# ReactiveBayes/RxInfer.jl

Hardware: NVIDIA H100
Metric: gaussian_messages_per_sec_batched_lgssm_d4_T1000 (higher is better)
Workload: dtype f32

## Files before the change

rxinfer.jl_b200/csrc/rxg_gain.cuh:

```cuda
#pragma once
#include <cooperative_groups.h>

#include "rxg_lgssm_common.cuh"

namespace rxg {
namespace cg = cooperative_groups;

constexpr int GS_CTAS = 8;
constexpr int GS_THREADS = 128;
constexpr int GS_NT = GS_CTAS * GS_THREADS;

struct ScanWs {
    double* fel;
    double* ftot;
    double* bel;
    double* btot;
};

template <int R, int C>
__device__ __forceinline__ Mat<double, R, C> ldcg_d(const double* p) {
    Mat<double, R, C> o;
#pragma unroll
    for (int i = 0; i < R * C; ++i) o.a[i] = __ldcg(p + i);
    return o;
}
template <int R, int C>
__device__ __forceinline__ Mat<double, R, C> ld_soa_d(const double* p, size_t n, size_t i) {
    Mat<double, R, C> o;
#pragma unroll
    for (int c = 0; c < R * C; ++c) o.a[c] = __ldcg(p + (size_t)c * n + i);
    return o;
}
template <int R, int C>
__device__ __forceinline__ void st_soa_d(double* p, size_t n, size_t i, const Mat<double, R, C>& A) {
#pragma unroll
    for (int c = 0; c < R * C; ++c) p[(size_t)c * n + i] = A.a[c];
}

template <int N, int K>
__device__ __forceinline__ Mat<double, N, K> solve_general(Mat<double, N, N> Mx, Mat<double, N, K> Rh) {
#pragma unroll
    for (int c = 0; c < N; ++c) {
        int p = c;
        double best = fabs(Mx(c, c));
#pragma unroll
        for (int r = c + 1; r < N; ++r) {
            const double v = fabs(Mx(r, c));
            if (v > best) { best = v; p = r; }
        }
#pragma unroll
        for (int r = c + 1; r < N; ++r) {
            if (r == p) {
#pragma unroll
                for (int j = c; j < N; ++j) { const double t = Mx(c, j); Mx(c, j) = Mx(r, j); Mx(r, j) = t; }
#pragma unroll
                for (int j = 0; j < K; ++j) { const double t = Rh(c, j); Rh(c, j) = Rh(r, j); Rh(r, j) = t; }
            }
        }
        const double inv = 1.0 / Mx(c, c);
#pragma unroll
        for (int r = c + 1; r < N; ++r) {
            const double f = Mx(r, c) * inv;
#pragma unroll
            for (int j = c + 1; j < N; ++j) Mx(r, j) = fma(-f, Mx(c, j), Mx(r, j));
#pragma unroll
            for (int j = 0; j < K; ++j) Rh(r, j) = fma(-f, Rh(c, j), Rh(r, j));
        }
    }
    Mat<double, N, K> X;
#pragma unroll
    for (int c = N - 1; c >= 0; --c) {
        const double inv = 1.0 / Mx(c, c);
#pragma unroll
        for (int k = 0; k < K; ++k) {
            double s = Rh(c, k);
#pragma unroll
            for (int j = c + 1; j < N; ++j) s = fma(-Mx(c, j), X(j, k), s);
            X(c, k) = s * inv;
        }
    }
    return X;
}

template <int D>
struct FwdEl {
    Mat<double, D, D> A, C, J;
};
template <int D>
struct BwdEl {
    Mat<double, D, D> E, L;
};

template <int D>
__device__ __forceinline__ FwdEl<D> fwd_identity() {
    FwdEl<D> e;
    e.A = identity<double, D>();
#pragma unroll
    for (int i = 0; i < D * D; ++i) { e.C.a[i] = 0.0; e.J.a[i] = 0.0; }
    return e;
}
template <int D>
__device__ __forceinline__ void fwd_store(double* p, size_t n, size_t i, const FwdEl<D>& e) {
    st_soa_d<D, D>(p, n, i, e.A);
    st_soa_d<D, D>(p + (size_t)D * D * n, n, i, e.C);
    st_soa_d<D, D>(p + (size_t)2 * D * D * n, n, i, e.J);
}
template <int D>
__device__ __forceinline__ FwdEl<D> fwd_load(const double* p, size_t n, size_t i) {
    FwdEl<D> e;
    e.A = ld_soa_d<D, D>(p, n, i);
    e.C = ld_soa_d<D, D>(p + (size_t)D * D * n, n, i);
    e.J = ld_soa_d<D, D>(p + (size_t)2 * D * D * n, n, i);
    return e;
}
template <int D, bool C_ONLY>
__device__ __forceinline__ FwdEl<D> fwd_combine(const FwdEl<D>& ei, const FwdEl<D>& ej) {
    Mat<double, D, D> Mx = mul(ei.C, ej.J);
#pragma unroll
    for (int i = 0; i < D; ++i) Mx(i, i) += 1.0;
    Mat<double, D, 2 * D> Rh;
#pragma unroll
    for (int i = 0; i < D; ++i)
#pragma unroll
        for (int j = 0; j < D; ++j) { Rh(i, j) = ei.A(i, j); Rh(i, D + j) = ei.C(i, j); }
    Mat<double, D, 2 * D> X = solve_general<D, 2 * D>(Mx, Rh);
    Mat<double, D, D> X1, X2;
#pragma unroll
    for (int i = 0; i < D; ++i)
#pragma unroll
        for (int j = 0; j < D; ++j) { X1(i, j) = X(i, j); X2(i, j) = X(i, D + j); }
    FwdEl<D> o;
    Mat<double, D, D> T2 = mul(ej.A, X2);
    o.C = sym_mul_nt_add(T2, ej.A, ej.C);
    if (!C_ONLY) {
        o.A = mul(ej.A, X1);
        Mat<double, D, D> JX = mul(ej.J, X1);
        Mat<double, D, D> AtJX = mul_tn(ei.A, JX);
#pragma unroll
        for (int i = 0; i < D; ++i)
#pragma unroll
            for (int j = 0; j <= i; ++j) {
                const double s = 0.5 * (AtJX(i, j) + AtJX(j, i)) + ei.J(i, j);
                o.J(i, j) = s; o.J(j, i) = s;
            }
    }
    return o;
}

template <int D>
__device__ __forceinline__ void bwd_store(double* p, size_t n, size_t i, const BwdEl<D>& e) {
    st_soa_d<D, D>(p, n, i, e.E);
    st_soa_d<D, D>(p + (size_t)D * D * n, n, i, e.L);
}
template <int D>
__device__ __forceinline__ BwdEl<D> bwd_load(const double* p, size_t n, size_t i) {
    BwdEl<D> e;
    e.E = ld_soa_d<D, D>(p, n, i);
    e.L = ld_soa_d<D, D>(p + (size_t)D * D * n, n, i);
    return e;
}
template <int D, bool L_ONLY>
__device__ __forceinline__ BwdEl<D> bwd_combine(const BwdEl<D>& early, const BwdEl<D>& late) {
    BwdEl<D> o;
    Mat<double, D, D> EL = mul(early.E, late.L);
    o.L = sym_mul_nt_add(EL, early.E, early.L);
    if (!L_ONLY) o.E = mul(early.E, late.E);
    return o;
}

template <int D, int M>
__global__ void __cluster_dims__(GS_CTAS, 1, 1) __launch_bounds__(GS_THREADS, 1)
gain_scan_kernel(const __grid_constant__ ModelF<D, M> mdl, GainWs ws, ScanWs sw, int T, int transition_first,
                 float* __restrict__ cov_shared_out, int* __restrict__ bad_out, const uint8_t* __restrict__ tmask,
                 const float* __restrict__ useq) {
    using TB = Tab<D, M>;
    cg::cluster_group cluster = cg::this_cluster();
    const int g = (int)cluster.block_rank() * GS_THREADS + (int)threadIdx.x;
    const int E = (T + GS_NT - 1) / GS_NT;
    const int k0 = g * E, k1 = min(k0 + E, T);
    constexpr int FE = 3 * D * D, BE = 2 * D * D;
    bool bad = false;

    const Mat<double, D, D> A = load_const<double, D, D>(mdl.A), P = load_const<double, D, D>(mdl.P);
    const Mat<double, M, D> B = load_const<double, M, D>(mdl.B);
    const Mat<double, M, M> Q = load_const<double, M, M>(mdl.Q);

    {
        FwdEl<D> acc = fwd_identity<D>();
        if (k0 < k1) {
            FwdEl<D> gen;
            {
                Mat<double, M, D> BP = mul(B, P);
                Mat<double, M, M> Sinn = sym_mul_nt_add(BP, B, Q);
                Chol<double, M> ch = cholesky<double, M, false>(Sinn, bad);
                Mat<double, D, M> V = solve_right_Lt(transpose(BP), ch.L);
                Mat<double, D, M> K = solve_right_L(V, ch.L);
                Mat<double, D, D> IKB = identity<double, D>();
#pragma unroll
                for (int i = 0; i < D; ++i)
#pragma unroll
                    for (int j = 0; j < D; ++j)
#pragma unroll
                        for (int k = 0; k < M; ++k) IKB(i, j) -= K(i, k) * B(k, j);
                gen.A = mul(IKB, A);
                gen.C = sym_downdate(P, V);
                Mat<double, M, D> BA = mul(B, A);
                Mat<double, M, D> Wm;
#pragma unroll
                for (int c = 0; c < D; ++c) {
                    Vec<double, M> col;
#pragma unroll
                    for (int r = 0; r < M; ++r) col(r) = BA(r, c);
                    Vec<double, M> z = solve_L(ch.L, col);
#pragma unroll
                    for (int r = 0; r < M; ++r) Wm(r, c) = z(r);
                }
                Mat<double, D, D> Z;
#pragma unroll
                for (int i = 0; i < D * D; ++i) Z.a[i] = 0.0;
                gen.J = sym_mul_nt_add(transpose(Wm), transpose(Wm), Z);
            }
            for (int k = k0; k < k1; ++k) {
                if (k == 0) {
                    Mat<double, D, D> S = load_const<double, D, D>(mdl.S0);
                    if (transition_first) { Mat<double, D, D> AS = mul(A, S); S = sym_mul_nt_add(AS, A, P); }
                    FwdEl<D> first;
#pragma unroll
                    for (int i = 0; i < D * D; ++i) { first.A.a[i] = 0.0; first.J.a[i] = 0.0; }
                    if (!tmask || tmask[0] != 0) {
                        Mat<double, M, D> BS = mul(B, S);
                        Mat<double, M, M> Sinn = sym_mul_nt_add(BS, B, Q);
                        Chol<double, M> ch = cholesky<double, M, false>(Sinn, bad);
                        Mat<double, D, M> V = solve_right_Lt(transpose(BS), ch.L);
                        first.C = sym_downdate(S, V);
                    } else {
                        first.C = S;
                    }
                    acc = first;
                } else {
                    const bool obs_k = !tmask || tmask[k] != 0;
                    if (obs_k) {
                        acc = (k == k0) ? gen : fwd_combine<D, false>(acc, gen);
                    } else {
                        FwdEl<D> miss;
                        miss.A = A; miss.C = P;
#pragma unroll
                        for (int i = 0; i < D * D; ++i) miss.J.a[i] = 0.0;
                        acc = (k == k0) ? miss : fwd_combine<D, false>(acc, miss);
                    }
                }
                if (E > 1) fwd_store<D>(sw.fel, T, k, acc);
            }
        }
        fwd_store<D>(sw.ftot, GS_NT, g, acc);
    }
    cluster.sync();
    int cur = 0;
    for (int off = 1; off < GS_NT; off <<= 1) {
        const double* src = sw.ftot + (size_t)cur * GS_NT * FE;
        double* dst = sw.ftot + (size_t)(cur ^ 1) * GS_NT * FE;
        FwdEl<D> mine = fwd_load<D>(src, GS_NT, g);
        if (g >= off && (g - off) * E < T && k0 < T) {
            FwdEl<D> prev = fwd_load<D>(src, GS_NT, g - off);
            mine = fwd_combine<D, false>(prev, mine);
        }
        fwd_store<D>(dst, GS_NT, g, mine);
        cluster.sync();
        cur ^= 1;
    }
    {
        const double* tot = sw.ftot + (size_t)cur * GS_NT * FE;
        if (E == 1) {
            if (g < T) store_d(ws.Sf + (size_t)g * D * D, ld_soa_d<D, D>(tot + (size_t)D * D * GS_NT, GS_NT, g));
        } else if (k0 < k1) {
            if (g == 0) {
                for (int k = k0; k < k1; ++k)
                    store_d(ws.Sf + (size_t)k * D * D, ld_soa_d<D, D>(sw.fel + (size_t)D * D * T, T, k));
            } else {
                const FwdEl<D> excl = fwd_load<D>(tot, GS_NT, g - 1);
                for (int k = k0; k < k1; ++k) {
                    const FwdEl<D> pk = fwd_load<D>(sw.fel, T, k);
                    store_d(ws.Sf + (size_t)k * D * D, fwd_combine<D, true>(excl, pk).C);
                }
            }
        }
    }
    cluster.sync();
    for (int t = g; t < T; t += GS_NT) {
        const Mat<double, D, D> Sf = ldcg_d<D, D>(ws.Sf + (size_t)t * D * D);
        Mat<double, D, D> Sp;
        if (t > 0) {
            Mat<double, D, D> Sfm = ldcg_d<D, D>(ws.Sf + (size_t)(t - 1) * D * D);
            Mat<double, D, D> AS = mul(A, Sfm);
            Sp = sym_mul_nt_add(AS, A, P);
        } else {
            Sp = load_const<double, D, D>(mdl.S0);
            if (transition_first) { Mat<double, D, D> AS = mul(A, Sp); Sp = sym_mul_nt_add(AS, A, P); }
        }
        const bool obs_t = !tmask || tmask[t] != 0;
        {
            Mat<double, D, M> K;
            Mat<double, M, M> Li;
            double cconst = 0.0;
#pragma unroll
            for (int i = 0; i < D * M; ++i) K.a[i] = 0.0;
#pragma unroll
            for (int i = 0; i < M * M; ++i) Li.a[i] = 0.0;
            if (obs_t) {
                Mat<double, M, D> BS = mul(B, Sp);
                Mat<double, M, M> Sinn = sym_mul_nt_add(BS, B, Q);
                Chol<double, M> ch = cholesky<double, M, true>(Sinn, bad);
                Mat<double, D, M> V = solve_right_Lt(transpose(BS), ch.L);
                K = solve_right_L(V, ch.L);
#pragma unroll
                for (int j = 0; j < M; ++j) {
                    Li(j, j) = ch.L(j, j);
// ... 2 lines not shown
                        double sacc = 0.0;
#pragma unroll
                        for (int k = j; k < i; ++k) sacc -= ch.L(i, k) * Li(k, j);
                        Li(i, j) = sacc * ch.L(i, i);
                    }
                }
                cconst = M * RXG_HALF_LOG_2PI - ch.neg_half_logdet;
            }
            Mat<double, D, D> IKB = identity<double, D>();
#pragma unroll
            for (int i = 0; i < D; ++i)
#pragma unroll
                for (int j = 0; j < D; ++j)
#pragma unroll
                    for (int k = 0; k < M; ++k) IKB(i, j) -= K(i, k) * B(k, j);
            Mat<double, D, D> F = (t > 0 || transition_first) ? mul(IKB, A) : IKB;
            float* rec = ws.fwd + (size_t)t * TB::FWD_REC;
            store_f(rec + TB::F_OFF, F);
            store_f(rec + TB::K_OFF, K);
            store_f(rec + TB::LI_OFF, Li);
            rec[TB::C_OFF] = (float)cconst;
            Vec<double, D> uu, gf;
#pragma unroll
            for (int i = 0; i < D; ++i) uu(i) = (double)(useq ? useq[(size_t)t * D + i] : mdl.u[i]);
            gf = mulv(IKB, uu);
            if (!(t > 0 || transition_first)) {
#pragma unroll
                for (int i = 0; i < D; ++i) gf(i) = 0.0;
            }
            store_fv(rec + TB::GF_OFF, gf);
            store_f(ws.sf + (size_t)t * TB::SF_REC, Sf);
        }
        float* brec = ws.bwd + (size_t)t * TB::BWD_REC;
        BwdEl<D> be;
        Vec<double, D> gb;
#pragma unroll
        for (int i = 0; i < D; ++i) gb(i) = 0.0;
        if (t < T - 1) {
            Mat<double, D, D> AS = mul(A, Sf);
            Mat<double, D, D> Sp1 = sym_mul_nt_add(AS, A, P);
            Chol<double, D> ch = cholesky<double, D, false>(Sp1, bad);
            Mat<double, D, D> U = solve_right_Lt(transpose(AS), ch.L);
            be.E = solve_right_L(U, ch.L);
            be.L = sym_downdate(Sf, U);
            Mat<double, D, D> Em = identity<double, D>();
            Mat<double, D, D> GA = mul(be.E, A);
#pragma unroll
            for (int i = 0; i < D * D; ++i) Em.a[i] -= GA.a[i];
            store_f(brec + TB::E_OFF, Em);
            store_f(brec + TB::G_OFF, be.E);
            Vec<double, D> uu;
#pragma unroll
            for (int i = 0; i < D; ++i) uu(i) = -(double)(useq ? useq[(size_t)(t + 1) * D + i] : mdl.u[i]);
            gb = mulv(be.E, uu);
        } else {
#pragma unroll
            for (int i = 0; i < D * D; ++i) be.E.a[i] = 0.0;
            be.L = Sf;
            store_f(brec + TB::E_OFF, identity<double, D>());
            store_f(brec + TB::G_OFF, be.E);
        }
        store_fv(brec + TB::GB_OFF, gb);
        bwd_store<D>(sw.bel, T, t, be);
    }
    cluster.sync();
    {
        BwdEl<D> acc;
        acc.E = identity<double, D>();
#pragma unroll
        for (int i = 0; i < D * D; ++i) acc.L.a[i] = 0.0;
        for (int r = k0; r < k1; ++r) {
            const int t = T - 1 - r;
            const BwdEl<D> el = bwd_load<D>(sw.bel, T, t);
            acc = (r == k0) ? el : bwd_combine<D, false>(el, acc);
            if (E > 1) bwd_store<D>(sw.bel, T, t, acc);
        }
        bwd_store<D>(sw.btot, GS_NT, g, acc);
    }
    cluster.sync();
    cur = 0;
    for (int off = 1; off < GS_NT; off <<= 1) {
        const double* src = sw.btot + (size_t)cur * GS_NT * BE;
        double* dst = sw.btot + (size_t)(cur ^ 1) * GS_NT * BE;
        BwdEl<D> mine = bwd_load<D>(src, GS_NT, g);
        if (g >= off && k0 < T) {
            BwdEl<D> prev = bwd_load<D>(src, GS_NT, g - off);
            mine = bwd_combine<D, false>(mine, prev);
        }
        bwd_store<D>(dst, GS_NT, g, mine);
        cluster.sync();
        cur ^= 1;
    }
    {
        const double* tot = sw.btot + (size_t)cur * GS_NT * BE;
        BwdEl<D> excl;
        if (E > 1 && g > 0 && k0 < k1) excl = bwd_load<D>(tot, GS_NT, g - 1);
        for (int r = k0; r < k1; ++r) {
            const int t = T - 1 - r;
            Mat<double, D, D> Ss;
            if (E == 1) {
                Ss = ld_soa_d<D, D>(tot + (size_t)D * D * GS_NT, GS_NT, g);
            } else {
                const BwdEl<D> pr = bwd_load<D>(sw.bel, T, t);
                Ss = (g == 0) ? pr.L : bwd_combine<D, true>(pr, excl).L;
            }
            store_f(ws.bwd + (size_t)t * TB::BWD_REC + TB::SS_OFF, Ss);
            if (cov_shared_out) store_f(cov_shared_out + (size_t)t * D * D, Ss);
        }
    }
    if (bad) atomicOr(bad_out, 1);
}

}
```

rxinfer.jl_b200/csrc/rxg_lgssm.cu:

```cuda
#include <math.h>
#include <stdlib.h>

#include <utility>

#include "rxg_chain_step.cuh"
#include "rxg_gain.cuh"
#include "rxg_internal.h"
#include "rxg_linalg.cuh"
#include "rxg_lgssm_cluster.cuh"
#include "rxg_lgssm_common.cuh"
#include "rxg_lgssm_shared.cuh"
#include "rxg_lgssm_seg.cuh"
#include "rxg_sweep_select.h"

namespace rxg {

template <int D, int M, bool PER_CHAIN, bool SMOOTH, bool USEQ = false>
__global__ void __launch_bounds__(128)
lgssm_chain_kernel(const __grid_constant__ ModelF<D, M> mdl, PerChainPtrs pc,
                   const float* __restrict__ y, const uint8_t* __restrict__ mask,
                   float* __restrict__ mean, float* __restrict__ cov, float* __restrict__ nle,
                   int32_t* __restrict__ status, int T, int64_t batch, int transition_first,
                   const float* __restrict__ useq = nullptr, int64_t ustride = 0, int uchain = 0) {
    const int64_t b = (int64_t)blockIdx.x * blockDim.x + threadIdx.x;
// ... 388 lines not shown
    launched = false;
    if constexpr (D * D <= 16 && M >= D) {
        using CT = ClusterTab<D, M>;
        bool offset = false;
        for (int i = 0; i < D; ++i) offset |= (mdl.u[i] != 0.f);
        const bool aligned = (((uintptr_t)c.y | (uintptr_t)c.mean | (uintptr_t)c.cov) & 15) == 0;
        if (!c.smooth || c.nle || c.useq || offset || c.mean0_chain || c.batch % 32 != 0 || !aligned ||
            ctx->opt[RXG_OPT_SWEEP_VARIANT] != 0 || ctx->opt[RXG_OPT_FORCE_CPT] != 0)
            return RXG_OK;
        const size_t smem = CT::smem_bytes(c.T);
        int smem_max = 0;
        RXG_CUDA(ctx, cudaDeviceGetAttribute(&smem_max, cudaDevAttrMaxSharedMemoryPerBlockOptin, ctx->device));
        if (smem > (size_t)smem_max) return RXG_OK;
        const bool peer = c.po.n_mean > 0 || c.po.n_cov > 0;
        auto kern = peer ? lgssm_cluster_sweep_kernel<D, M, true> : lgssm_cluster_sweep_kernel<D, M, false>;
        RXG_CUDA(ctx, cudaFuncSetAttribute(kern, cudaFuncAttributeMaxDynamicSharedMemorySize, (int)smem));
        cudaLaunchConfig_t cfg = {};
        cudaLaunchAttribute attr[1];
        attr[0].id = cudaLaunchAttributeClusterDimension;
        attr[0].val.clusterDim.x = CL_CTAS;
        attr[0].val.clusterDim.y = 1;
        attr[0].val.clusterDim.z = 1;
        cfg.gridDim = dim3((unsigned)(c.batch / 32 * CL_CTAS));
        cfg.blockDim = dim3(32 * CL_WARPS);
        cfg.dynamicSmemBytes = smem;
        cfg.stream = ctx->stream;
        cfg.attrs = attr;
        cfg.numAttrs = 1;
        int nclusters = 0;
        RXG_CUDA(ctx, cudaOccupancyMaxActiveClusters(&nclusters, kern, &cfg));
        if (nclusters < 1) return RXG_OK;

        const int spc = CT::spc(c.T);
        cluster_tables_kernel<D, M><<<1, 256, 0, ctx->stream>>>(ws, cl_tab, c.T, spc);
        if (ctx->profile) cudaEventRecord(ctx->ev[1], ctx->stream);
        RXG_CUDA(ctx, cudaLaunchKernelEx(&cfg, kern, (const float*)ws.fwd, (const float*)ws.bwd, (const float*)cl_tab, c.y,
                                         c.mean, c.cov, c.T, c.batch, write_cov, mdl, c.po));
        if (ctx->profile) cudaEventRecord(ctx->ev[2], ctx->stream);
        ctx->launches += 2;
        c.fused_peer_stores = peer;
        launched = true;
        return check_cuda(ctx, cudaGetLastError(), "lgssm_cluster_sweep_kernel launch");
    }
    return RXG_OK;
}

template <int D, int M>
static int run_shared_family(rxg_ctx* ctx, LgssmCall& c) {
    using TB = Tab<D, M>;
    ModelF<D, M> mdl = {};
    fill_model<D, M>(mdl, c);
    const size_t T = (size_t)c.T;
    size_t off = 0;
    auto carve = [&](size_t bytes) { size_t o = off; off += (bytes + 255) / 256 * 256; return o; };
    const size_t o_fwd = carve(T * TB::FWD_REC * sizeof(float));
    const size_t o_bwd = carve(T * TB::BWD_REC * sizeof(float));
    const size_t o_sf = carve(T * TB::SF_REC * sizeof(float));
    const size_t o_Sp = carve(T * D * D * sizeof(double));
    const size_t o_Sf = carve(T * D * D * sizeof(double));
    const size_t o_Cc = carve(T * D * D * sizeof(double));
    const size_t o_Gd = carve(T * D * D * sizeof(double));
    const size_t o_fel = carve(T * 3 * D * D * sizeof(double));
    const size_t o_ftot = carve((size_t)2 * GS_NT * 3 * D * D * sizeof(double));
    const size_t o_bel = carve(T * 2 * D * D * sizeof(double));
    const size_t o_btot = carve((size_t)2 * GS_NT * 2 * D * D * sizeof(double));
    using ST = SegTab<D, M>;
    const size_t nseg = (T + ST::L - 1) / ST::L;
    const size_t o_srec_t = carve(T * ST::REC * sizeof(float)), o_snrec = carve(T * ST::NREC * sizeof(float));
    const size_t o_ssrec = carve(nseg * ST::SREC * sizeof(float));
    const size_t o_ctab = carve(c.want_cov_table ? T * D * D * sizeof(float) : 0);
    const size_t o_cl = carve(ClusterTab<D, M>::table_floats(c.T) * sizeof(float));
    char* base = (char*)workspace(ctx, off);
    if (!base) return RXG_ERR_CUDA;
    GainWs ws;
    ws.fwd = (float*)(base + o_fwd); ws.bwd = (float*)(base + o_bwd); ws.sf = (float*)(base + o_sf);
    ws.Sp = (double*)(base + o_Sp); ws.Sf = (double*)(base + o_Sf);
    ws.Cc = (double*)(base + o_Cc); ws.Gd = (double*)(base + o_Gd);
    ScanWs sw;
    sw.fel = (double*)(base + o_fel); sw.ftot = (double*)(base + o_ftot);
    sw.bel = (double*)(base + o_bel); sw.btot = (double*)(base + o_btot);

    const int tf = (c.flags & RXG_TRANSITION_FIRST) ? 1 : 0;
    const bool cov_shared = (c.flags & RXG_COV_SHARED_OUT) != 0;
    c.cov_table = (c.want_cov_table && c.smooth) ? (float*)(base + o_ctab) : nullptr;
    if (ctx->profile) cudaEventRecord(ctx->ev[0], ctx->stream);
    float* cov_once = (cov_shared && c.cov && c.smooth) ? c.cov : (c.smooth ? c.cov_table : nullptr);
    const float* useq_tab = c.useq_chain ? nullptr : c.useq;
    if (ctx->opt[RXG_OPT_GAIN_SEQ] != 0) {
        gain_riccati_seq<D, M><<<1, 32, 0, ctx->stream>>>(mdl, ws, c.T, tf, bad_flag(ctx), c.tmask);
        gain_tables<D, M><<<(c.T + 63) / 64, 64, 0, ctx->stream>>>(mdl, ws, c.T, tf, bad_flag(ctx), c.tmask, useq_tab);
        ctx->launches += 2;
        if (c.smooth) {
            gain_smooth_seq<D, M><<<1, 32, 0, ctx->stream>>>(ws, c.T, cov_once);
            ctx->launches += 1;
        }
    } else {
        gain_scan_kernel<D, M><<<GS_CTAS, GS_THREADS, 0, ctx->stream>>>(mdl, ws, sw, c.T, tf, cov_once, bad_flag(ctx), c.tmask,
                                                                          useq_tab);
        ctx->launches += 1;
    }
    if (!c.smooth && cov_shared && c.cov) {
        const int n = c.T * D * D;
        copy_table_kernel<<<(n + 255) / 256, 256, 0, ctx->stream>>>(ws.sf, TB::SF_REC, D * D, c.T, c.cov);
        ctx->launches += 1;
    }
    int rc = check_cuda(ctx, cudaGetLastError(), "gain table kernels launch");
    if (rc != RXG_OK) return rc;
    if (c.ev_tables) RXG_CUDA(ctx, cudaEventRecord(c.ev_tables, ctx->stream));
    if (c.tables_only) return RXG_OK;
    const int write_cov = (c.cov != nullptr && !cov_shared) ? 1 : 0;
    bool launched = false;
    rc = launch_cluster_if_eligible<D, M>(ctx, c, mdl, ws, (float*)(base + o_cl), write_cov, launched);
    if (rc != RXG_OK || launched) return rc;
    const long long variant = ctx->opt[RXG_OPT_SWEEP_VARIANT];
    if (variant == 3 && !c.useq && seg_sweep_eligible<D, M>(c)) {
        SegWs sgw;
        sgw.rec = (float*)(base + o_srec_t); sgw.nrec = (float*)(base + o_snrec); sgw.srec = (float*)(base + o_ssrec);
        return launch_seg<D, M>(ctx, c, mdl, ws, sgw, write_cov, variant == 3);
    }
    SweepQuery q = {};
    q.d = D;
    q.m = M;
    q.batch = c.batch;
    q.sm_count = ctx->sm_count;
    q.force_cpt = ctx->opt[RXG_OPT_FORCE_CPT];
    q.aligned16 = (((uintptr_t)c.y | (uintptr_t)c.mean | (uintptr_t)c.cov | (uintptr_t)c.nle | (uintptr_t)c.mean0_chain |
                    (uintptr_t)(c.useq_chain ? c.useq : nullptr)) & 15) == 0;
    q.smooth = c.smooth;
    q.evid = c.nle != nullptr;
    for (int i = 0; i < D; ++i) q.offset |= (mdl.u[i] != 0.f);
    q.input = !c.useq ? InputSeq::none : (c.useq_chain ? InputSeq::per_chain : InputSeq::shared);
// ... 56 lines not shown
```

rxinfer.jl_b200/csrc/rxg_lgssm_cluster.cuh:

```cuda
#pragma once
#include <cooperative_groups.h>

#include "rxg_lgssm_common.cuh"
#include "rxg_lgssm_shared.cuh"

namespace rxg {

constexpr int CL_CTAS = 8;
constexpr int CL_WARPS = 8;
constexpr int CL_L = 16;

template <int D, int M>
struct ClusterTab {
    static constexpr int FK = pad4(D * D) + pad4(D * M);
    static constexpr int EG = 2 * pad4(D * D);
    static constexpr int REC = 2 * pad4(D * D);
    static constexpr int PSI_OFF = pad4(D * D);
    static_assert(Tab<D, M>::F_OFF == 0 && Tab<D, M>::K_OFF == pad4(D * D) && Tab<D, M>::E_OFF == 0 &&
                      Tab<D, M>::G_OFF == pad4(D * D),
                  "the staged prefixes are the first FK / EG floats of the gain records");

    static __host__ __device__ int spc(int T) { return ((T + CL_L - 1) / CL_L + CL_CTAS - 1) / CL_CTAS; }
    static size_t table_floats(int T) { return (size_t)(CL_CTAS * spc(T) + CL_CTAS) * REC; }
    static size_t smem_bytes(int T) {
        const size_t S = (size_t)spc(T) * CL_L;
        return 4 * (S * (M * 32 + FK + EG) + (size_t)(spc(T) + CL_CTAS) * REC + (size_t)spc(T) * D * 32 + 2 * D * 32);
    }
};

template <int D, int M>
__global__ void __launch_bounds__(256) cluster_tables_kernel(GainWs ws, float* __restrict__ tab, int T, int spc) {
    using TB = Tab<D, M>;
    using CT = ClusterTab<D, M>;
    const int nsub = CL_CTAS * spc;
    for (int j = threadIdx.x; j < nsub; j += blockDim.x) {
        const int a = j * CL_L, e = min(a + CL_L, T);
        Mat<double, D, D> Phi = identity<double, D>(), Psi = identity<double, D>();
        for (int t = a; t < e; ++t) {
            Phi = mul(load_const<double, D, D>(ws.fwd + (size_t)t * TB::FWD_REC + TB::F_OFF), Phi);
            Psi = mul(Psi, load_const<double, D, D>(ws.bwd + (size_t)t * TB::BWD_REC + TB::G_OFF));
        }
        store_f(tab + (size_t)j * CT::REC, Phi);
        store_f(tab + (size_t)j * CT::REC + CT::PSI_OFF, Psi);
    }
    __syncthreads();
    for (int r = threadIdx.x; r < CL_CTAS; r += blockDim.x) {
        Mat<double, D, D> Phi = identity<double, D>(), Psi = identity<double, D>();
        for (int j = r * spc; j < (r + 1) * spc; ++j) {
            Phi = mul(load_const<double, D, D>(tab + (size_t)j * CT::REC), Phi);
            Psi = mul(Psi, load_const<double, D, D>(tab + (size_t)j * CT::REC + CT::PSI_OFF));
        }
        store_f(tab + (size_t)(nsub + r) * CT::REC, Phi);
        store_f(tab + (size_t)(nsub + r) * CT::REC + CT::PSI_OFF, Psi);
    }
}

template <int D>
__device__ __forceinline__ void affine_step(const float* Mx, float (&v)[D], const float (&w)[D]) {
    float Mr[pad4(D * D)];
    load_smem<pad4(D * D)>(Mx, Mr);
    float n[D];
#pragma unroll
    for (int i = 0; i < D; ++i) {
        float a = w[i];
#pragma unroll
        for (int j = 0; j < D; ++j) a = __fmaf_rn(Mr[i * D + j], v[j], a);
        n[i] = a;
    }
#pragma unroll
    for (int i = 0; i < D; ++i) v[i] = n[i];
}

template <int D, int M>
__device__ __forceinline__ void store_cov_span(const float* __restrict__ bwd_tab, float* __restrict__ cov, int64_t batch,
                                               int T) {
    using TB = Tab<D, M>;
    constexpr int NT = 32 * CL_WARPS;
    const int n4 = (int)(batch / 4);
    const int span = D * D * T;
    const int64_t base = (int64_t)blockIdx.x * span;
    float4* out = reinterpret_cast<float4*>(cov) + base;
    const int step_rows = NT / n4, step_cols = NT % n4;
    int i = (int)threadIdx.x;
    const int64_t q = base + i;
    int row = (int)(q / n4), col = (int)(q - (int64_t)row * n4);
    int cur = -1;
// ... 268 lines not shown
```

Baseline: 149.9 billion.

## Move gain-scan carries to shared memory with DSMEM cluster exclusive; parallelize table products

Result: faster. 152.3 billion, median of 6 (+1.6%).

```diff
diff --git a/rxinfer.jl_b200/csrc/rxg_gain.cuh b/rxinfer.jl_b200/csrc/rxg_gain.cuh
--- a/rxinfer.jl_b200/csrc/rxg_gain.cuh
+++ b/rxinfer.jl_b200/csrc/rxg_gain.cuh
@@ -12,10 +12,13 @@
 
 struct ScanWs {
     double* fel;
-    double* ftot;
     double* bel;
-    double* btot;
 };
+
+template <int D>
+constexpr size_t gain_scan_smem_bytes() {
+    return sizeof(double) * (size_t)(3 * D * D) * (2 * GS_THREADS + 3 + GS_CTAS);
+}
 
 template <int R, int C>
 __device__ __forceinline__ Mat<double, R, C> ldcg_d(const double* p) {
@@ -24,18 +27,40 @@
     for (int i = 0; i < R * C; ++i) o.a[i] = __ldcg(p + i);
     return o;
 }
-template <int R, int C>
-__device__ __forceinline__ Mat<double, R, C> ld_soa_d(const double* p, size_t n, size_t i) {
-    Mat<double, R, C> o;
-#pragma unroll
-    for (int c = 0; c < R * C; ++c) o.a[c] = __ldcg(p + (size_t)c * n + i);
-    return o;
-}
-template <int R, int C>
-__device__ __forceinline__ void st_soa_d(double* p, size_t n, size_t i, const Mat<double, R, C>& A) {
-#pragma unroll
-    for (int c = 0; c < R * C; ++c) p[(size_t)c * n + i] = A.a[c];
-}
+
+template <int D, bool GMEM>
+struct ElRef {
+    double* p;
+    size_t n;
+    __device__ __forceinline__ double get(int c) const {
+        if constexpr (GMEM) return __ldcg(p + (size_t)c * n);
+        else return p[(size_t)c * n];
+    }
+    __device__ __forceinline__ Mat<double, D, D> part(int q) const {
+        Mat<double, D, D> o;
+#pragma unroll
+        for (int c = 0; c < D * D; ++c) o.a[c] = get(q * D * D + c);
+        return o;
+    }
+    __device__ __forceinline__ void put(int q, const Mat<double, D, D>& X) const {
+#pragma unroll
+        for (int c = 0; c < D * D; ++c) p[(size_t)(q * D * D + c) * n] = X.a[c];
+    }
+    template <int NP>
+    __device__ __forceinline__ void copy_from(const ElRef<D, true>& s) const {
+#pragma unroll
+        for (int c = 0; c < NP * D * D; ++c) p[(size_t)c * n] = s.get(c);
+    }
+    template <int NP>
+    __device__ __forceinline__ void copy_from(const ElRef<D, false>& s) const {
+#pragma unroll
+        for (int c = 0; c < NP * D * D; ++c) p[(size_t)c * n] = s.get(c);
+    }
+};
+template <int D>
+using SRef = ElRef<D, false>;
+template <int D>
+using GRef = ElRef<D, true>;
 
 template <int N, int K>
 __device__ __forceinline__ Mat<double, N, K> solve_general(Mat<double, N, N> Mx, Mat<double, N, K> Rh) {
@@ -85,87 +110,147 @@
 template <int D>
 struct FwdEl {
     Mat<double, D, D> A, C, J;
+    __device__ __forceinline__ void put(int q, const Mat<double, D, D>& X) { (q == 0 ? A : q == 1 ? C : J) = X; }
 };
 template <int D>
 struct BwdEl {
     Mat<double, D, D> E, L;
+    __device__ __forceinline__ void put(int q, const Mat<double, D, D>& X) { (q == 0 ? E : L) = X; }
 };
-
-template <int D>
-__device__ __forceinline__ FwdEl<D> fwd_identity() {
-    FwdEl<D> e;
-    e.A = identity<double, D>();
-#pragma unroll
-    for (int i = 0; i < D * D; ++i) { e.C.a[i] = 0.0; e.J.a[i] = 0.0; }
-    return e;
-}
-template <int D>
-__device__ __forceinline__ void fwd_store(double* p, size_t n, size_t i, const FwdEl<D>& e) {
-    st_soa_d<D, D>(p, n, i, e.A);
-    st_soa_d<D, D>(p + (size_t)D * D * n, n, i, e.C);
-    st_soa_d<D, D>(p + (size_t)2 * D * D * n, n, i, e.J);
-}
-template <int D>
-__device__ __forceinline__ FwdEl<D> fwd_load(const double* p, size_t n, size_t i) {
-    FwdEl<D> e;
-    e.A = ld_soa_d<D, D>(p, n, i);
-    e.C = ld_soa_d<D, D>(p + (size_t)D * D * n, n, i);
-    e.J = ld_soa_d<D, D>(p + (size_t)2 * D * D * n, n, i);
-    return e;
-}
-template <int D, bool C_ONLY>
-__device__ __forceinline__ FwdEl<D> fwd_combine(const FwdEl<D>& ei, const FwdEl<D>& ej) {
-    Mat<double, D, D> Mx = mul(ei.C, ej.J);
-#pragma unroll
-    for (int i = 0; i < D; ++i) Mx(i, i) += 1.0;
-    Mat<double, D, 2 * D> Rh;
+template <int D>
+struct OnlyPart {
+    Mat<double, D, D> X;
+    __device__ __forceinline__ void put(int, const Mat<double, D, D>& Y) { X = Y; }
+};
+
+template <int D, bool C_ONLY, class EI, class EJ, class OUT>
+__device__ __forceinline__ void fwd_combine(const EI& ei, const EJ& ej, OUT& out) {
+    Mat<double, D, 2 * D> X;
+    {
+        Mat<double, D, D> Mx = mul(ei.part(1), ej.part(2));
+#pragma unroll
+        for (int i = 0; i < D; ++i) Mx(i, i) += 1.0;
+        Mat<double, D, 2 * D> Rh;
+        {
+            const Mat<double, D, D> Ai = ei.part(0), Ci = ei.part(1);
+#pragma unroll
+            for (int i = 0; i < D; ++i)
+#pragma unroll
+                for (int j = 0; j < D; ++j) { Rh(i, j) = Ai(i, j); Rh(i, D + j) = Ci(i, j); }
+        }
+        X = solve_general<D, 2 * D>(Mx, Rh);
+    }
+    Mat<double, D, D> X1, X2;
 #pragma unroll
     for (int i = 0; i < D; ++i)
 #pragma unroll
-        for (int j = 0; j < D; ++j) { Rh(i, j) = ei.A(i, j); Rh(i, D + j) = ei.C(i, j); }
-    Mat<double, D, 2 * D> X = solve_general<D, 2 * D>(Mx, Rh);
-    Mat<double, D, D> X1, X2;
-#pragma unroll
-    for (int i = 0; i < D; ++i)
-#pragma unroll
         for (int j = 0; j < D; ++j) { X1(i, j) = X(i, j); X2(i, j) = X(i, D + j); }
-    FwdEl<D> o;
-    Mat<double, D, D> T2 = mul(ej.A, X2);
-    o.C = sym_mul_nt_add(T2, ej.A, ej.C);
     if (!C_ONLY) {
-        o.A = mul(ej.A, X1);
-        Mat<double, D, D> JX = mul(ej.J, X1);
-        Mat<double, D, D> AtJX = mul_tn(ei.A, JX);
+        Mat<double, D, D> JX = mul(ej.part(2), X1);
+        Mat<double, D, D> AtJX = mul_tn(ei.part(0), JX);
+        const Mat<double, D, D> Ji = ei.part(2);
+        Mat<double, D, D> oJ;
 #pragma unroll
         for (int i = 0; i < D; ++i)
 #pragma unroll
             for (int j = 0; j <= i; ++j) {
-                const double s = 0.5 * (AtJX(i, j) + AtJX(j, i)) + ei.J(i, j);
-                o.J(i, j) = s; o.J(j, i) = s;
-            }
-    }
-    return o;
-}
-
-template <int D>
-__device__ __forceinline__ void bwd_store(double* p, size_t n, size_t i, const BwdEl<D>& e) {
-    st_soa_d<D, D>(p, n, i, e.E);
-    st_soa_d<D, D>(p + (size_t)D * D * n, n, i, e.L);
-}
-template <int D>
-__device__ __forceinline__ BwdEl<D> bwd_load(const double* p, size_t n, size_t i) {
-    BwdEl<D> e;
-    e.E = ld_soa_d<D, D>(p, n, i);
-    e.L = ld_soa_d<D, D>(p + (size_t)D * D * n, n, i);
-    return e;
-}
-template <int D, bool L_ONLY>
-__device__ __forceinline__ BwdEl<D> bwd_combine(const BwdEl<D>& early, const BwdEl<D>& late) {
-    BwdEl<D> o;
-    Mat<double, D, D> EL = mul(early.E, late.L);
-    o.L = sym_mul_nt_add(EL, early.E, early.L);
-    if (!L_ONLY) o.E = mul(early.E, late.E);
-    return o;
+                const double s = 0.5 * (AtJX(i, j) + AtJX(j, i)) + Ji(i, j);
+                oJ(i, j) = s; oJ(j, i) = s;
+            }
+        out.put(2, oJ);
+    }
+    {
+        const Mat<double, D, D> Aj = ej.part(0);
+        Mat<double, D, D> T2 = mul(Aj, X2);
+        out.put(1, sym_mul_nt_add(T2, Aj, ej.part(1)));
+    }
+    if (!C_ONLY) out.put(0, mul(ej.part(0), X1));
+}
+
+template <int D, bool L_ONLY, class EE, class EL, class OUT>
+__device__ __forceinline__ void bwd_combine(const EE& early, const EL& late, OUT& out) {
+    {
+        const Mat<double, D, D> Ee = early.part(0);
+        Mat<double, D, D> ELm = mul(Ee, late.part(1));
+        out.put(1, sym_mul_nt_add(ELm, Ee, early.part(1)));
+    }
+    if (!L_ONLY) out.put(0, mul(early.part(0), late.part(0)));
+}
+
+template <int D>
+__device__ __noinline__ void fwd_combine_full(double* ei, int ni, double* ej, int nj, double* out, int no) {
+    const SRef<D> a{ei, (size_t)ni}, b{ej, (size_t)nj}, o{out, (size_t)no};
+    fwd_combine<D, false>(a, b, o);
+}
+template <int D>
+__device__ __noinline__ void bwd_combine_full(double* early, int ne, double* late, int nl, double* out, int no) {
+    const SRef<D> a{early, (size_t)ne}, b{late, (size_t)nl}, o{out, (size_t)no};
+    bwd_combine<D, false>(a, b, o);
+}
+template <int D, bool GI, bool GJ, bool GO>
+__device__ __forceinline__ void fwd_full(const ElRef<D, GI>& a, const ElRef<D, GJ>& b, const ElRef<D, GO>& o) {
+    fwd_combine_full<D>(a.p, (int)a.n, b.p, (int)b.n, o.p, (int)o.n);
+}
+template <int D, bool GI, bool GJ, bool GO>
+__device__ __forceinline__ void bwd_full(const ElRef<D, GI>& a, const ElRef<D, GJ>& b, const ElRef<D, GO>& o) {
+    bwd_combine_full<D>(a.p, (int)a.n, b.p, (int)b.n, o.p, (int)o.n);
+}
+
+template <int D, bool FWD>
+__device__ __forceinline__ double* cta_scan(double* s0, double* s1, int n) {
+    constexpr int NE = (FWD ? 3 : 2) * D * D;
+    const int i = (int)threadIdx.x;
+    double* src = s0;
+    double* dst = s1;
+    for (int off = 1; off < n; off <<= 1) {
+        const SRef<D> mine{src + i, GS_THREADS}, out{dst + i, GS_THREADS};
+        if (i >= off && i < n) {
+            const SRef<D> prev{src + i - off, GS_THREADS};
+            if constexpr (FWD) fwd_full<D>(prev, mine, out);
+            else bwd_full<D>(mine, prev, out);
+        } else if (i < n) {
+            out.template copy_from<NE / (D * D)>(mine);
+        }
+        __syncthreads();
+        double* t = src; src = dst; dst = t;
+    }
+    return src;
+}
+
+template <int D, bool FWD>
+__device__ __forceinline__ void cluster_exclusive(cg::cluster_group& cluster, double* stot, double* sx, int r) {
+    constexpr int NE = (FWD ? 3 : 2) * D * D;
+    for (int idx = (int)threadIdx.x; idx < r * NE; idx += GS_THREADS) {
+        const int j = idx / NE, c = idx - j * NE;
+        const double* src = cluster.map_shared_rank(stot, FWD ? j : r - 1 - j);
+        sx[j * NE + c] = src[c];
+    }
+    __syncthreads();
+    for (int off = 1; off < r; off <<= 1) {
+        const int j = 2 * off * (int)threadIdx.x;
+        if (j + off < r) {
+            const SRef<D> a{sx + j * NE, 1}, b{sx + (j + off) * NE, 1};
+            if constexpr (FWD) fwd_full<D>(a, b, a);
+            else bwd_full<D>(a, b, a);
+        }
+        __syncthreads();
+    }
+}
+
+template <int D, bool FWD>
+__device__ __forceinline__ void store_cta_total(const double* s, int n, double* stot) {
+    constexpr int NE = (FWD ? 3 : 2) * D * D;
+    const int c = (int)threadIdx.x;
+    if (c < NE) {
+        double v;
+        if (n > 0) {
+            v = s[(size_t)c * GS_THREADS + n - 1];
+        } else {
+            const int q = c / (D * D), e = c % (D * D);
+            v = (q == 0 && e / D == e % D) ? 1.0 : 0.0;
+        }
+        stot[c] = v;
+    }
 }
 
 template <int D, int M>
@@ -174,114 +259,115 @@
                  float* __restrict__ cov_shared_out, int* __restrict__ bad_out, const uint8_t* __restrict__ tmask,
                  const float* __restrict__ useq) {
     using TB = Tab<D, M>;
+    constexpr int FE = 3 * D * D;
+    extern __shared__ double gs_smem[];
+    double* sel = gs_smem;
+    double* sel1 = sel + FE * GS_THREADS;
+    double* sgen = sel1 + FE * GS_THREADS;
+    double* smiss = sgen + FE;
+    double* stot = smiss + FE;
+    double* sx = stot + FE;
+
     cg::cluster_group cluster = cg::this_cluster();
-    const int g = (int)cluster.block_rank() * GS_THREADS + (int)threadIdx.x;
+    const int r = (int)cluster.block_rank();
+    const int tid = (int)threadIdx.x;
+    const int g = r * GS_THREADS + tid;
     const int E = (T + GS_NT - 1) / GS_NT;
     const int k0 = g * E, k1 = min(k0 + E, T);
-    constexpr int FE = 3 * D * D, BE = 2 * D * D;
+    const int nact = max(0, min(GS_THREADS, (T + E - 1) / E - r * GS_THREADS));
     bool bad = false;
 
     const Mat<double, D, D> A = load_const<double, D, D>(mdl.A), P = load_const<double, D, D>(mdl.P);
     const Mat<double, M, D> B = load_const<double, M, D>(mdl.B);
     const Mat<double, M, M> Q = load_const<double, M, M>(mdl.Q);
 
-    {
-        FwdEl<D> acc = fwd_identity<D>();
-        if (k0 < k1) {
-            FwdEl<D> gen;
-            {
-                Mat<double, M, D> BP = mul(B, P);
-                Mat<double, M, M> Sinn = sym_mul_nt_add(BP, B, Q);
+    if (tid == 0) {
+        FwdEl<D> gen;
+        Mat<double, M, D> BP = mul(B, P);
+        Mat<double, M, M> Sinn = sym_mul_nt_add(BP, B, Q);
+        Chol<double, M> ch = cholesky<double, M, false>(Sinn, bad);
+        Mat<double, D, M> V = solve_right_Lt(transpose(BP), ch.L);
+        Mat<double, D, M> K = solve_right_L(V, ch.L);
+        Mat<double, D, D> IKB = identity<double, D>();
+#pragma unroll
+        for (int i = 0; i < D; ++i)
+#pragma unroll
+            for (int j = 0; j < D; ++j)
+#pragma unroll
+                for (int k = 0; k < M; ++k) IKB(i, j) -= K(i, k) * B(k, j);
+        gen.A = mul(IKB, A);
+        gen.C = sym_downdate(P, V);
+        Mat<double, M, D> BA = mul(B, A);
+        Mat<double, M, D> Wm;
+#pragma unroll
+        for (int c = 0; c < D; ++c) {
+            Vec<double, M> col;
+#pragma unroll
+            for (int rr = 0; rr < M; ++rr) col(rr) = BA(rr, c);
+            Vec<double, M> z = solve_L(ch.L, col);
+#pragma unroll
+            for (int rr = 0; rr < M; ++rr) Wm(rr, c) = z(rr);
+        }
+        Mat<double, D, D> Z;
+#pragma unroll
+        for (int i = 0; i < D * D; ++i) Z.a[i] = 0.0;
+        gen.J = sym_mul_nt_add(transpose(Wm), transpose(Wm), Z);
+        const SRef<D> sg{sgen, 1}, sm{smiss, 1};
+        sg.put(0, gen.A); sg.put(1, gen.C); sg.put(2, gen.J);
+        sm.put(0, A); sm.put(1, P); sm.put(2, Z);
+    }
+    __syncthreads();
+    const SRef<D> mine{sel + tid, GS_THREADS};
+    for (int k = k0; k < k1; ++k) {
+        if (k == 0) {
+            Mat<double, D, D> S = load_const<double, D, D>(mdl.S0);
+            if (transition_first) { Mat<double, D, D> AS = mul(A, S); S = sym_mul_nt_add(AS, A, P); }
+            Mat<double, D, D> Z;
+#pragma unroll
+            for (int i = 0; i < D * D; ++i) Z.a[i] = 0.0;
+            if (!tmask || tmask[0] != 0) {
+                Mat<double, M, D> BS = mul(B, S);
+                Mat<double, M, M> Sinn = sym_mul_nt_add(BS, B, Q);
                 Chol<double, M> ch = cholesky<double, M, false>(Sinn, bad);
-                Mat<double, D, M> V = solve_right_Lt(transpose(BP), ch.L);
-                Mat<double, D, M> K = solve_right_L(V, ch.L);
-                Mat<double, D, D> IKB = identity<double, D>();
-#pragma unroll
-                for (int i = 0; i < D; ++i)
-#pragma unroll
-                    for (int j = 0; j < D; ++j)
-#pragma unroll
-                        for (int k = 0; k < M; ++k) IKB(i, j) -= K(i, k) * B(k, j);
-                gen.A = mul(IKB, A);
-                gen.C = sym_downdate(P, V);
-                Mat<double, M, D> BA = mul(B, A);
-                Mat<double, M, D> Wm;
-#pragma unroll
-                for (int c = 0; c < D; ++c) {
-                    Vec<double, M> col;
-#pragma unroll
-                    for (int r = 0; r < M; ++r) col(r) = BA(r, c);
-                    Vec<double, M> z = solve_L(ch.L, col);
-#pragma unroll
-                    for (int r = 0; r < M; ++r) Wm(r, c) = z(r);
-                }
-                Mat<double, D, D> Z;
-#pragma unroll
-                for (int i = 0; i < D * D; ++i) Z.a[i] = 0.0;
-                gen.J = sym_mul_nt_add(transpose(Wm), transpose(Wm), Z);
-            }
+                Mat<double, D, M> V = solve_right_Lt(transpose(BS), ch.L);
+                mine.put(1, sym_downdate(S, V));
+            } else {
+                mine.put(1, S);
+            }
+            mine.put(0, Z);
+            mine.put(2, Z);
+        } else {
+            const SRef<D> el{(!tmask || tmask[k] != 0) ? sgen : smiss, 1};
+            if (k == k0) mine.template copy_from<3>(el);
+            else fwd_full<D>(mine, el, mine);
+        }
+        if (E > 1) GRef<D>{sw.fel + k, (size_t)T}.template copy_from<3>(mine);
+    }
+    __syncthreads();
+    double* fin = cta_scan<D, true>(sel, sel1, nact);
+    const SRef<D> pre{fin + tid, GS_THREADS};
+    store_cta_total<D, true>(fin, nact, stot);
+    cluster.sync();
+    if (r > 0 && nact > 0) {
+        cluster_exclusive<D, true>(cluster, stot, sx, r);
+        if (tid < nact) {
+            const SRef<D> ex{sx, 1};
+            fwd_full<D>(ex, pre, pre);
+        }
+        __syncthreads();
+    }
+    if (E == 1) {
+        if (g < T) store_d(ws.Sf + (size_t)g * D * D, pre.part(1));
+    } else if (k0 < k1) {
+        if (g == 0) {
+            for (int k = k0; k < k1; ++k)
+                store_d(ws.Sf + (size_t)k * D * D, GRef<D>{sw.fel + k, (size_t)T}.part(1));
+        } else {
+            const SRef<D> excl = tid > 0 ? SRef<D>{fin + tid - 1, GS_THREADS} : SRef<D>{sx, 1};
             for (int k = k0; k < k1; ++k) {
-                if (k == 0) {
-                    Mat<double, D, D> S = load_const<double, D, D>(mdl.S0);
-                    if (transition_first) { Mat<double, D, D> AS = mul(A, S); S = sym_mul_nt_add(AS, A, P); }
-                    FwdEl<D> first;
-#pragma unroll
-                    for (int i = 0; i < D * D; ++i) { first.A.a[i] = 0.0; first.J.a[i] = 0.0; }
-                    if (!tmask || tmask[0] != 0) {
-                        Mat<double, M, D> BS = mul(B, S);
-                        Mat<double, M, M> Sinn = sym_mul_nt_add(BS, B, Q);
-                        Chol<double, M> ch = cholesky<double, M, false>(Sinn, bad);
-                        Mat<double, D, M> V = solve_right_Lt(transpose(BS), ch.L);
-                        first.C = sym_downdate(S, V);
-                    } else {
-                        first.C = S;
-                    }
-                    acc = first;
-                } else {
-                    const bool obs_k = !tmask || tmask[k] != 0;
-                    if (obs_k) {
-                        acc = (k == k0) ? gen : fwd_combine<D, false>(acc, gen);
-                    } else {
-                        FwdEl<D> miss;
-                        miss.A = A; miss.C = P;
-#pragma unroll
-                        for (int i = 0; i < D * D; ++i) miss.J.a[i] = 0.0;
-                        acc = (k == k0) ? miss : fwd_combine<D, false>(acc, miss);
-                    }
-                }
-                if (E > 1) fwd_store<D>(sw.fel, T, k, acc);
-            }
-        }
-        fwd_store<D>(sw.ftot, GS_NT, g, acc);
-    }
-    cluster.sync();
-    int cur = 0;
-    for (int off = 1; off < GS_NT; off <<= 1) {
-        const double* src = sw.ftot + (size_t)cur * GS_NT * FE;
-        double* dst = sw.ftot + (size_t)(cur ^ 1) * GS_NT * FE;
-        FwdEl<D> mine = fwd_load<D>(src, GS_NT, g);
-        if (g >= off && (g - off) * E < T && k0 < T) {
-            FwdEl<D> prev = fwd_load<D>(src, GS_NT, g - off);
-            mine = fwd_combine<D, false>(prev, mine);
-        }
-        fwd_store<D>(dst, GS_NT, g, mine);
-        cluster.sync();
-        cur ^= 1;
-    }
-    {
-        const double* tot = sw.ftot + (size_t)cur * GS_NT * FE;
-        if (E == 1) {
-            if (g < T) store_d(ws.Sf + (size_t)g * D * D, ld_soa_d<D, D>(tot + (size_t)D * D * GS_NT, GS_NT, g));
-        } else if (k0 < k1) {
-            if (g == 0) {
-                for (int k = k0; k < k1; ++k)
-                    store_d(ws.Sf + (size_t)k * D * D, ld_soa_d<D, D>(sw.fel + (size_t)D * D * T, T, k));
-            } else {
-                const FwdEl<D> excl = fwd_load<D>(tot, GS_NT, g - 1);
-                for (int k = k0; k < k1; ++k) {
-                    const FwdEl<D> pk = fwd_load<D>(sw.fel, T, k);
-                    store_d(ws.Sf + (size_t)k * D * D, fwd_combine<D, true>(excl, pk).C);
-                }
+                OnlyPart<D> o;
+                fwd_combine<D, true>(excl, GRef<D>{sw.fel + k, (size_t)T}, o);
+                store_d(ws.Sf + (size_t)k * D * D, o.X);
             }
         }
     }
@@ -350,7 +436,7 @@
             store_f(ws.sf + (size_t)t * TB::SF_REC, Sf);
         }
         float* brec = ws.bwd + (size_t)t * TB::BWD_REC;
-        BwdEl<D> be;
+        const GRef<D> bel{sw.bel + t, (size_t)T};
         Vec<double, D> gb;
 #pragma unroll
         for (int i = 0; i < D; ++i) gb(i) = 0.0;
@@ -359,74 +445,71 @@
             Mat<double, D, D> Sp1 = sym_mul_nt_add(AS, A, P);
             Chol<double, D> ch = cholesky<double, D, false>(Sp1, bad);
             Mat<double, D, D> U = solve_right_Lt(transpose(AS), ch.L);
-            be.E = solve_right_L(U, ch.L);
-            be.L = sym_downdate(Sf, U);
+            const Mat<double, D, D> G = solve_right_L(U, ch.L);
+            bel.put(0, G);
+            bel.put(1, sym_downdate(Sf, U));
             Mat<double, D, D> Em = identity<double, D>();
-            Mat<double, D, D> GA = mul(be.E, A);
+            Mat<double, D, D> GA = mul(G, A);
 #pragma unroll
             for (int i = 0; i < D * D; ++i) Em.a[i] -= GA.a[i];
             store_f(brec + TB::E_OFF, Em);
-            store_f(brec + TB::G_OFF, be.E);
+            store_f(brec + TB::G_OFF, G);
             Vec<double, D> uu;
 #pragma unroll
             for (int i = 0; i < D; ++i) uu(i) = -(double)(useq ? useq[(size_t)(t + 1) * D + i] : mdl.u[i]);
-            gb = mulv(be.E, uu);
+            gb = mulv(G, uu);
         } else {
-#pragma unroll
-            for (int i = 0; i < D * D; ++i) be.E.a[i] = 0.0;
-            be.L = Sf;
+            Mat<double, D, D> Z;
+#pragma unroll
+            for (int i = 0; i < D * D; ++i) Z.a[i] = 0.0;
+            bel.put(0, Z);
+            bel.put(1, Sf);
             store_f(brec + TB::E_OFF, identity<double, D>());
-            store_f(brec + TB::G_OFF, be.E);
+            store_f(brec + TB::G_OFF, Z);
         }
         store_fv(brec + TB::GB_OFF, gb);
-        bwd_store<D>(sw.bel, T, t, be);
     }
     cluster.sync();
-    {
-        BwdEl<D> acc;
-        acc.E = identity<double, D>();
-#pragma unroll
-        for (int i = 0; i < D * D; ++i) acc.L.a[i] = 0.0;
-        for (int r = k0; r < k1; ++r) {
-            const int t = T - 1 - r;
-            const BwdEl<D> el = bwd_load<D>(sw.bel, T, t);
-            acc = (r == k0) ? el : bwd_combine<D, false>(el, acc);
-            if (E > 1) bwd_store<D>(sw.bel, T, t, acc);
-        }
-        bwd_store<D>(sw.btot, GS_NT, g, acc);
-    }
+    for (int q = k0; q < k1; ++q) {
+        const GRef<D> el{sw.bel + (T - 1 - q), (size_t)T};
+        if (q == k0) mine.template copy_from<2>(el);
+        else bwd_full<D>(el, mine, mine);
+        if (E > 1) el.template copy_from<2>(mine);
+    }
+    __syncthreads();
+    fin = cta_scan<D, false>(sel, sel1, nact);
+    store_cta_total<D, false>(fin, nact, stot);
     cluster.sync();
-    cur = 0;
-    for (int off = 1; off < GS_NT; off <<= 1) {
-        const double* src = sw.btot + (size_t)cur * GS_NT * BE;
-        double* dst = sw.btot + (size_t)(cur ^ 1) * GS_NT * BE;
-        BwdEl<D> mine = bwd_load<D>(src, GS_NT, g);
-        if (g >= off && k0 < T) {
-            BwdEl<D> prev = bwd_load<D>(src, GS_NT, g - off);
-            mine = bwd_combine<D, false>(mine, prev);
-        }
-        bwd_store<D>(dst, GS_NT, g, mine);
-        cluster.sync();
-        cur ^= 1;
-    }
-    {
-        const double* tot = sw.btot + (size_t)cur * GS_NT * BE;
-        BwdEl<D> excl;
-        if (E > 1 && g > 0 && k0 < k1) excl = bwd_load<D>(tot, GS_NT, g - 1);
-        for (int r = k0; r < k1; ++r) {
-            const int t = T - 1 - r;
-            Mat<double, D, D> Ss;
-            if (E == 1) {
-                Ss = ld_soa_d<D, D>(tot + (size_t)D * D * GS_NT, GS_NT, g);
+    if (r > 0 && nact > 0) {
+        cluster_exclusive<D, false>(cluster, stot, sx, r);
+        if (tid < nact) {
+            const SRef<D> ex{sx, 1}, suf{fin + tid, GS_THREADS};
+            bwd_full<D>(suf, ex, suf);
+        }
+        __syncthreads();
+    }
+    cluster.barrier_arrive();
+    for (int q = k0; q < k1; ++q) {
+        const int t = T - 1 - q;
+        Mat<double, D, D> Ss;
+        if (E == 1) {
+            Ss = SRef<D>{fin + tid, GS_THREADS}.part(1);
+        } else {
+            const GRef<D> pr{sw.bel + t, (size_t)T};
+            if (g == 0) {
+                Ss = pr.part(1);
             } else {
-                const BwdEl<D> pr = bwd_load<D>(sw.bel, T, t);
-                Ss = (g == 0) ? pr.L : bwd_combine<D, true>(pr, excl).L;
-            }
-            store_f(ws.bwd + (size_t)t * TB::BWD_REC + TB::SS_OFF, Ss);
-            if (cov_shared_out) store_f(cov_shared_out + (size_t)t * D * D, Ss);
-        }
+                const SRef<D> excl = tid > 0 ? SRef<D>{fin + tid - 1, GS_THREADS} : SRef<D>{sx, 1};
+                OnlyPart<D> o;
+                bwd_combine<D, true>(pr, excl, o);
+                Ss = o.X;
+            }
+        }
+        store_f(ws.bwd + (size_t)t * TB::BWD_REC + TB::SS_OFF, Ss);
+        if (cov_shared_out) store_f(cov_shared_out + (size_t)t * D * D, Ss);
     }
     if (bad) atomicOr(bad_out, 1);
-}
-
-}
+    cluster.barrier_wait();
+}
+
+}
diff --git a/rxinfer.jl_b200/csrc/rxg_lgssm.cu b/rxinfer.jl_b200/csrc/rxg_lgssm.cu
--- a/rxinfer.jl_b200/csrc/rxg_lgssm.cu
+++ b/rxinfer.jl_b200/csrc/rxg_lgssm.cu
@@ -444,7 +444,8 @@
         if (nclusters < 1) return RXG_OK;
 
         const int spc = CT::spc(c.T);
-        cluster_tables_kernel<D, M><<<1, 256, 0, ctx->stream>>>(ws, cl_tab, c.T, spc);
+        cluster_tables_kernel<D, M><<<1, CT_THREADS, (size_t)CL_CTAS * spc * CT::REC * sizeof(float), ctx->stream>>>(
+            ws, cl_tab, c.T, spc);
         if (ctx->profile) cudaEventRecord(ctx->ev[1], ctx->stream);
         RXG_CUDA(ctx, cudaLaunchKernelEx(&cfg, kern, (const float*)ws.fwd, (const float*)ws.bwd, (const float*)cl_tab, c.y,
                                          c.mean, c.cov, c.T, c.batch, write_cov, mdl, c.po));
@@ -473,9 +474,7 @@
     const size_t o_Cc = carve(T * D * D * sizeof(double));
     const size_t o_Gd = carve(T * D * D * sizeof(double));
     const size_t o_fel = carve(T * 3 * D * D * sizeof(double));
-    const size_t o_ftot = carve((size_t)2 * GS_NT * 3 * D * D * sizeof(double));
     const size_t o_bel = carve(T * 2 * D * D * sizeof(double));
-    const size_t o_btot = carve((size_t)2 * GS_NT * 2 * D * D * sizeof(double));
     using ST = SegTab<D, M>;
     const size_t nseg = (T + ST::L - 1) / ST::L;
     const size_t o_srec_t = carve(T * ST::REC * sizeof(float)), o_snrec = carve(T * ST::NREC * sizeof(float));
@@ -489,8 +488,8 @@
     ws.Sp = (double*)(base + o_Sp); ws.Sf = (double*)(base + o_Sf);
     ws.Cc = (double*)(base + o_Cc); ws.Gd = (double*)(base + o_Gd);
     ScanWs sw;
-    sw.fel = (double*)(base + o_fel); sw.ftot = (double*)(base + o_ftot);
-    sw.bel = (double*)(base + o_bel); sw.btot = (double*)(base + o_btot);
+    sw.fel = (double*)(base + o_fel);
+    sw.bel = (double*)(base + o_bel);
 
     const int tf = (c.flags & RXG_TRANSITION_FIRST) ? 1 : 0;
     const bool cov_shared = (c.flags & RXG_COV_SHARED_OUT) != 0;
@@ -507,8 +506,10 @@
             ctx->launches += 1;
         }
     } else {
-        gain_scan_kernel<D, M><<<GS_CTAS, GS_THREADS, 0, ctx->stream>>>(mdl, ws, sw, c.T, tf, cov_once, bad_flag(ctx), c.tmask,
-                                                                          useq_tab);
+        constexpr size_t smem = gain_scan_smem_bytes<D>();
+        RXG_CUDA(ctx, cudaFuncSetAttribute(gain_scan_kernel<D, M>, cudaFuncAttributeMaxDynamicSharedMemorySize, (int)smem));
+        gain_scan_kernel<D, M><<<GS_CTAS, GS_THREADS, smem, ctx->stream>>>(mdl, ws, sw, c.T, tf, cov_once, bad_flag(ctx),
+                                                                             c.tmask, useq_tab);
         ctx->launches += 1;
     }
     if (!c.smooth && cov_shared && c.cov) {
diff --git a/rxinfer.jl_b200/csrc/rxg_lgssm_cluster.cuh b/rxinfer.jl_b200/csrc/rxg_lgssm_cluster.cuh
--- a/rxinfer.jl_b200/csrc/rxg_lgssm_cluster.cuh
+++ b/rxinfer.jl_b200/csrc/rxg_lgssm_cluster.cuh
@@ -28,30 +28,63 @@
     }
 };
 
+template <int D>
+constexpr int ct_group() { return D * D <= 1 ? 1 : D * D <= 4 ? 4 : 16; }
+constexpr int CT_THREADS = 1024;
+
+template <int D, int GS>
+__device__ __forceinline__ double ct_mul_entry(unsigned mask, double x, double y, int i, int j) {
+    double s = __shfl_sync(mask, x, i * D, GS) * __shfl_sync(mask, y, j, GS);
+#pragma unroll
+    for (int k = 1; k < D; ++k) s = fma(__shfl_sync(mask, x, i * D + k, GS), __shfl_sync(mask, y, k * D + j, GS), s);
+    return s;
+}
+
 template <int D, int M>
-__global__ void __launch_bounds__(256) cluster_tables_kernel(GainWs ws, float* __restrict__ tab, int T, int spc) {
+__global__ void __launch_bounds__(CT_THREADS) cluster_tables_kernel(GainWs ws, float* __restrict__ tab, int T, int spc) {
     using TB = Tab<D, M>;
     using CT = ClusterTab<D, M>;
+    constexpr int GS = ct_group<D>();
+    constexpr int NG = CT_THREADS / GS;
+    extern __shared__ float ct_sub[];
     const int nsub = CL_CTAS * spc;
-    for (int j = threadIdx.x; j < nsub; j += blockDim.x) {
-        const int a = j * CL_L, e = min(a + CL_L, T);
-        Mat<double, D, D> Phi = identity<double, D>(), Psi = identity<double, D>();
-        for (int t = a; t < e; ++t) {
-            Phi = mul(load_const<double, D, D>(ws.fwd + (size_t)t * TB::FWD_REC + TB::F_OFF), Phi);
-            Psi = mul(Psi, load_const<double, D, D>(ws.bwd + (size_t)t * TB::BWD_REC + TB::G_OFF));
-        }
-        store_f(tab + (size_t)j * CT::REC, Phi);
-        store_f(tab + (size_t)j * CT::REC + CT::PSI_OFF, Psi);
-    }
-    __syncthreads();
-    for (int r = threadIdx.x; r < CL_CTAS; r += blockDim.x) {
-        Mat<double, D, D> Phi = identity<double, D>(), Psi = identity<double, D>();
-        for (int j = r * spc; j < (r + 1) * spc; ++j) {
-            Phi = mul(load_const<double, D, D>(tab + (size_t)j * CT::REC), Phi);
-            Psi = mul(Psi, load_const<double, D, D>(tab + (size_t)j * CT::REC + CT::PSI_OFF));
-        }
-        store_f(tab + (size_t)(nsub + r) * CT::REC, Phi);
-        store_f(tab + (size_t)(nsub + r) * CT::REC + CT::PSI_OFF, Psi);
+    const int lane = (int)threadIdx.x % GS, q = min(lane, D * D - 1), i = q / D, j = q % D;
+    const bool owner = lane < D * D;
+    const unsigned mask = (GS == 32 ? 0xffffffffu : (1u << GS) - 1u) << ((int)threadIdx.x % 32 / GS * GS);
+    for (int task = (int)threadIdx.x / GS; task < 2 * nsub; task += NG) {
+        const int sub = task >> 1;
+        const bool psi = task & 1;
+        const int a = sub * CL_L, e = min(a + CL_L, T);
+        const float* rec = psi ? ws.bwd + TB::G_OFF : ws.fwd + TB::F_OFF;
+        const size_t stride = psi ? TB::BWD_REC : TB::FWD_REC;
+        float r[CL_L];
+#pragma unroll
+        for (int l = 0; l < CL_L; ++l) r[l] = a + l < e ? rec[(size_t)(a + l) * stride + q] : 0.f;
+        double v = i == j ? 1.0 : 0.0;
+#pragma unroll
+        for (int l = 0; l < CL_L; ++l) {
+            const double x = (double)r[l];
+            const double n = ct_mul_entry<D, GS>(mask, psi ? v : x, psi ? x : v, i, j);
+            if (a + l < e) v = n;
+        }
+        if (owner) {
+            const size_t o = (size_t)sub * CT::REC + (psi ? CT::PSI_OFF : 0) + q;
+            tab[o] = (float)v;
+            ct_sub[o] = (float)v;
+        }
+    }
+    __syncthreads();
+    const int task = (int)threadIdx.x / GS;
+    if (task < 2 * CL_CTAS) {
+        const int sl = task >> 1;
+        const bool psi = task & 1;
+        const int off = psi ? CT::PSI_OFF : 0;
+        double v = i == j ? 1.0 : 0.0;
+        for (int s = sl * spc; s < (sl + 1) * spc; ++s) {
+            const double x = (double)ct_sub[(size_t)s * CT::REC + off + q];
+            v = ct_mul_entry<D, GS>(mask, psi ? v : x, psi ? x : v, i, j);
+        }
+        if (owner) tab[(size_t)(nsub + sl) * CT::REC + off + q] = (float)v;
     }
 }
 
```
